# szabodabo/CUDA-MPI-Reductions

Measured on AMD Instinct MI355X. Metric: reduction bandwidth (GB/s, whole node), 1B-double sum at 1/2/4/8 MI355X, higher is better.
Workload: dtype fp64; 1 GPU; global_batch=1000000000, seq_len=1, parallelism=dp1, backend=nccl, n_total_elements=1000000000, op=SUM, collective=fused, launch=graph (chunk 871, 1 replays)

## Files before the change

### csrc/include/mireduce/direct.hpp

```cpp
#pragma once

#include <hip/hip_runtime_api.h>

#include <array>
#include <cstddef>
#include <cstdint>
#include <vector>

#include "mireduce/types.hpp"
#include "mireduce/xrank.hpp"

namespace mireduce {

constexpr int kMaxDirectRanks = 16;
constexpr int kMaxDirectBlocks = 1024;
constexpr int kDirectBlock = 512;
constexpr int kDirectPhases = 3;

struct DirectDesc {
  const char* in[kMaxDirectRanks];
  char* out[kMaxDirectRanks];
  unsigned* sig[kMaxDirectRanks];
  unsigned* ctl;
  int rank;
  int world;
  uint64_t timeout_ticks;
};

class DirectAllreduce {
 public:
  DirectAllreduce(int device, size_t bytes, int grid = 0, double timeout_s = 10.0);
  ~DirectAllreduce();
  DirectAllreduce(const DirectAllreduce&) = delete;
  DirectAllreduce& operator=(const DirectAllreduce&) = delete;

  static constexpr size_t kHandleBytes = 3 * sizeof(IpcHandleBytes) + sizeof(int32_t);
  std::vector<char> handles() const;
  void connect(int rank, int world, const std::vector<std::vector<char>>& all);

  void* in() const { return in_; }
  void* out() const { return out_; }
  size_t bytes() const { return bytes_; }
  int grid() const { return grid_; }
  int rank() const { return rank_; }
  int world() const { return world_; }
  bool connected() const { return connected_; }

  void allreduce(size_t count, DType t, Op op, hipStream_t s);
  void reduce(size_t count, DType t, Op op, int root, hipStream_t s);
  void read_peers(size_t bytes_each, hipStream_t s);
  unsigned error() const;
  unsigned epoch() const;

 private:
  void launch(size_t count, DType t, Op op, int gather_rank, hipStream_t s);
  int device_ = 0, rank_ = 0, world_ = 1, grid_ = 0;
  size_t bytes_ = 0;
  double timeout_s_ = 10.0;
  bool connected_ = false;
  void* in_ = nullptr;
  void* out_ = nullptr;
  unsigned* sig_ = nullptr;
  unsigned* ctl_ = nullptr;
  DirectDesc* desc_ = nullptr;
  uint32_t* sink_ = nullptr;
  std::vector<void*> opened_;
  std::vector<const void*> peer_in_;
};

void direct_chunk(size_t count, size_t elem_size, int world, int r, size_t* begin, size_t* end);

}
```

### csrc/kernels/direct.hip

```cpp
#include <hip/hip_runtime.h>

#include <algorithm>
#include <cstdint>
#include <cstring>

#include "mireduce/check.hpp"
#include "mireduce/direct.hpp"
#include "mireduce/peer.hpp"
#include "mireduce/ops.hpp"

namespace mireduce {
namespace kern {

__device__ __forceinline__ void peer_barrier(const DirectDesc* d, int phase, unsigned e, unsigned err,
                                             bool release) {
  asm volatile("s_waitcnt vmcnt(0)" ::: "memory");
  __syncthreads();
  if (threadIdx.x < 64) {
    const int lane = threadIdx.x;
    if (release) __builtin_amdgcn_fence(__ATOMIC_RELEASE, "");
    const int world = d->world;
    const uint64_t slot = (static_cast<uint64_t>(phase) * kMaxDirectBlocks + blockIdx.x) * kMaxDirectRanks;
    if (lane < world) {
      __hip_atomic_store(d->sig[lane] + slot + d->rank, e, __ATOMIC_RELAXED, __HIP_MEMORY_SCOPE_SYSTEM);
      const unsigned* mine = d->sig[d->rank] + slot + lane;
      const uint64_t limit = err ? 0 : d->timeout_ticks;
      const uint64_t t0 = static_cast<uint64_t>(wall_clock64());
      while (__hip_atomic_load(mine, __ATOMIC_RELAXED, __HIP_MEMORY_SCOPE_SYSTEM) != e) {
        if (static_cast<uint64_t>(wall_clock64()) - t0 > limit) {
          __hip_atomic_fetch_or(d->ctl + 1, 1u, __ATOMIC_RELAXED, __HIP_MEMORY_SCOPE_AGENT);
          break;
        }
        __builtin_amdgcn_s_sleep(1);
      }
    }
    __builtin_amdgcn_fence(__ATOMIC_ACQUIRE, "");
  }
  __syncthreads();
}

__device__ __forceinline__ void block_range(uint64_t nvec, uint64_t* v0, uint64_t* v1) {
  const uint64_t per = (nvec + gridDim.x - 1) / gridDim.x;
  *v0 = std::min<uint64_t>(nvec, blockIdx.x * per);
  *v1 = std::min<uint64_t>(nvec, *v0 + per);
}

template <class T>
__device__ __forceinline__ uint64_t chunk_elems(uint64_t count, int world) {
  constexpr uint64_t N = 16 / sizeof(T);
  const uint64_t per = (count + world - 1) / world;
  return (per + N - 1) / N * N;
}

template <int W>
constexpr int direct_unroll() {
  return W >= 4 ? 1 : (W >= 2 ? 2 : 4);
}

template <class OpT, class T, int W>
__global__ __launch_bounds__(kDirectBlock) void direct_kernel(const DirectDesc* __restrict__ d, uint64_t count,
                                                               int gather_rank) {
  constexpr int N = 16 / sizeof(T);
  constexpr int U = W > 0 ? direct_unroll<W>() : 1;
  using V = T __attribute__((ext_vector_type(N)));
  __shared__ unsigned s_epoch, s_err;
  if (threadIdx.x == 0) {
    s_epoch = __hip_atomic_load(d->ctl, __ATOMIC_RELAXED, __HIP_MEMORY_SCOPE_AGENT) + 1u;
    s_err = __hip_atomic_load(d->ctl + 1, __ATOMIC_RELAXED, __HIP_MEMORY_SCOPE_AGENT);
  }
  __syncthreads();
  const unsigned e = s_epoch;
  const int world = W > 0 ? W : d->world;
  const int rank = d->rank;

  peer_barrier(d, 0, e, s_err, true);

  const uint64_t per = chunk_elems<T>(count, world);
  const uint64_t perv = per / N;
  uint64_t v0, v1;
  block_range(perv, &v0, &v1);
  {
    const uint64_t cb = std::min<uint64_t>(count, rank * per);
    const uint64_t ce = std::min<uint64_t>(count, cb + per);
    const uint64_t nvec = (ce - cb) / N;
    const uint64_t r1 = std::min(v1, nvec);
    T* out = reinterpret_cast<T*>(d->out[rank]);
    if constexpr (W > 0) {
      for (uint64_t i0 = v0 + threadIdx.x; i0 < r1; i0 += U * kDirectBlock) {
        V v[U][W];
#pragma unroll
        for (int u = 0; u < U; ++u) {
          const uint64_t i = i0 + static_cast<uint64_t>(u) * kDirectBlock;
          if (i < r1)
#pragma unroll
            for (int p = 0; p < W; ++p)
              v[u][p] = __builtin_nontemporal_load(reinterpret_cast<const V*>(d->in[p]) + cb / N + i);
        }
#pragma unroll
        for (int u = 0; u < U; ++u) {
          const uint64_t i = i0 + static_cast<uint64_t>(u) * kDirectBlock;
          if (i >= r1) continue;
          V acc = v[u][0];
#pragma unroll
          for (int p = 1; p < W; ++p)
#pragma unroll
            for (int k = 0; k < N; ++k) acc[k] = OpT::apply(acc[k], v[u][p][k]);
          reinterpret_cast<V*>(out)[cb / N + i] = acc;
        }
      }
    } else {
      for (uint64_t i = v0 + threadIdx.x; i < r1; i += kDirectBlock) {
        const uint64_t off = cb / N + i;
        V acc = __builtin_nontemporal_load(reinterpret_cast<const V*>(d->in[0]) + off);
        for (int p = 1; p < world; ++p) {
          const V v = __builtin_nontemporal_load(reinterpret_cast<const V*>(d->in[p]) + off);
#pragma unroll
          for (int k = 0; k < N; ++k) acc[k] = OpT::apply(acc[k], v[k]);
        }
        reinterpret_cast<V*>(out)[off] = acc;
      }
    }
    if (blockIdx.x == gridDim.x - 1) {
      for (uint64_t i = cb + nvec * N + threadIdx.x; i < ce; i += kDirectBlock) {
        T acc = reinterpret_cast<const T*>(d->in[0])[i];
        for (int p = 1; p < world; ++p) acc = OpT::apply(acc, reinterpret_cast<const T*>(d->in[p])[i]);
        out[i] = acc;
      }
    }
  }

  peer_barrier(d, 1, e, s_err, true);

  if (gather_rank < 0 || gather_rank == rank) {
    T* mine = reinterpret_cast<T*>(d->out[rank]);
    if constexpr (W > 0) {
      uint64_t nv[W];
#pragma unroll
      for (int p = 0; p < W; ++p) {
        const uint64_t b = std::min<uint64_t>(count, p * per);
        nv[p] = p == rank ? 0 : (std::min<uint64_t>(count, b + per) - b) / N;
      }
      for (uint64_t i0 = v0 + threadIdx.x; i0 < v1; i0 += U * kDirectBlock) {
        V v[U][W];
#pragma unroll
        for (int u = 0; u < U; ++u) {
          const uint64_t i = i0 + static_cast<uint64_t>(u) * kDirectBlock;
#pragma unroll
          for (int p = 0; p < W; ++p)
            if (i < v1 && i < nv[p])
              v[u][p] = __builtin_nontemporal_load(reinterpret_cast<const V*>(d->out[p]) + p * perv + i);
        }
#pragma unroll
        for (int u = 0; u < U; ++u) {
          const uint64_t i = i0 + static_cast<uint64_t>(u) * kDirectBlock;
#pragma unroll
          for (int p = 0; p < W; ++p)
            if (i < v1 && i < nv[p]) reinterpret_cast<V*>(mine)[p * perv + i] = v[u][p];
        }
      }
    } else {
      for (int p = 0; p < world; ++p) {
        if (p == rank) continue;
        const uint64_t b = std::min<uint64_t>(count, p * per);
        const uint64_t n = (std::min<uint64_t>(count, b + per) - b) / N;
        const uint64_t e1 = std::min(v1, n);
        for (uint64_t i = v0 + threadIdx.x; i < e1; i += kDirectBlock)
          reinterpret_cast<V*>(mine)[p * perv + i] = __builtin_nontemporal_load(reinterpret_cast<const V*>(d->out[p]) + p * perv + i);
      }
    }
    if (blockIdx.x == gridDim.x - 1) {
      for (int p = 0; p < world; ++p) {
        if (p == rank) continue;
        const uint64_t b = std::min<uint64_t>(count, p * per);
        const uint64_t e1 = std::min<uint64_t>(count, b + per);
        for (uint64_t i = b + (e1 - b) / N * N + threadIdx.x; i < e1; i += kDirectBlock)
          mine[i] = reinterpret_cast<const T*>(d->out[p])[i];
      }
    }
  }

  peer_barrier(d, 2, e, s_err, false);
  if (threadIdx.x == 0) {
    const unsigned prev = __hip_atomic_fetch_add(d->ctl + 2, 1u, __ATOMIC_RELAXED, __HIP_MEMORY_SCOPE_AGENT);
    if (prev == gridDim.x - 1) {
      __hip_atomic_store(d->ctl + 2, 0u, __ATOMIC_RELAXED, __HIP_MEMORY_SCOPE_AGENT);
      __hip_atomic_store(d->ctl, e, __ATOMIC_RELAXED, __HIP_MEMORY_SCOPE_AGENT);
    }
  }
}

}

void direct_chunk(size_t count, size_t elem_size, int world, int r, size_t* begin, size_t* end) {
  const size_t vec = 16 / elem_size;
  size_t per = (count + world - 1) / world;
  per = (per + vec - 1) / vec * vec;
  *begin = std::min(count, static_cast<size_t>(r) * per);
  *end = std::min(count, static_cast<size_t>(r + 1) * per);
}

namespace {

struct DeviceGuard {
  int prev = 0;
  explicit DeviceGuard(int dev) {
    MIREDUCE_HIP_THROW(hipGetDevice(&prev));
    MIREDUCE_HIP_THROW(hipSetDevice(dev));
  }
  ~DeviceGuard() { (void)hipSetDevice(prev); }
};

constexpr size_t kSigBytes = static_cast<size_t>(kDirectPhases) * kMaxDirectBlocks * kMaxDirectRanks * sizeof(unsigned);

using DirectFn = void (*)(const DirectDesc*, uint64_t, int, int, hipStream_t);

template <class OpT, class T, int W>
void launch_w(const DirectDesc* d, uint64_t count, int gather, int grid, hipStream_t s) {
  hipLaunchKernelGGL((kern::direct_kernel<OpT, T, W>), dim3(grid), dim3(kDirectBlock), 0, s, d, count, gather);
}

template <class OpT, class T>
DirectFn pick_world(int world) {
  switch (world) {
    case 1: return launch_w<OpT, T, 1>;
    case 2: return launch_w<OpT, T, 2>;
    case 3: return launch_w<OpT, T, 3>;
    case 4: return launch_w<OpT, T, 4>;
    case 5: return launch_w<OpT, T, 5>;
    case 6: return launch_w<OpT, T, 6>;
    case 7: return launch_w<OpT, T, 7>;
    case 8: return launch_w<OpT, T, 8>;
    default: return launch_w<OpT, T, 0>;
  }
}

template <class OpT>
DirectFn pick_type(DType t, int world) {
  switch (t) {
    case DType::Int32: return pick_world<OpT, int32_t>(world);
    case DType::Int64: return pick_world<OpT, int64_t>(world);
    case DType::Float32: return pick_world<OpT, float>(world);
    case DType::Float64: return pick_world<OpT, double>(world);
    default: MIREDUCE_REQUIRE(false, "direct: int32, int64, float32 or float64 only");
  }
  return nullptr;
}

}

DirectAllreduce::DirectAllreduce(int device, size_t bytes, int grid, double timeout_s) : timeout_s_(timeout_s) {
  MIREDUCE_REQUIRE(timeout_s > 0, "direct: timeout must be positive");
  if (device < 0) MIREDUCE_HIP_THROW(hipGetDevice(&device));
  device_ = device;
  DeviceGuard g(device_);
  int cus = 0;
  MIREDUCE_HIP_THROW(hipDeviceGetAttribute(&cus, hipDeviceAttributeMultiprocessorCount, device_));
  grid_ = grid > 0 ? grid : std::max(1, cus);
  MIREDUCE_REQUIRE(grid_ <= kMaxDirectBlocks, "direct: grid exceeds kMaxDirectBlocks");
  bytes_ = (std::max<size_t>(bytes, 16) + 255) / 256 * 256;
  MIREDUCE_HIP_THROW(hipExtMallocWithFlags(&in_, bytes_, hipDeviceMallocFinegrained));
  MIREDUCE_HIP_THROW(hipExtMallocWithFlags(&out_, bytes_, hipDeviceMallocFinegrained));
  MIREDUCE_HIP_THROW(hipExtMallocWithFlags(reinterpret_cast<void**>(&sig_), kSigBytes, hipDeviceMallocUncached));
  MIREDUCE_HIP_THROW(hipMemset(sig_, 0, kSigBytes));
  MIREDUCE_HIP_THROW(hipMalloc(reinterpret_cast<void**>(&ctl_), 256));
  MIREDUCE_HIP_THROW(hipMemset(ctl_, 0, 256));
  MIREDUCE_HIP_THROW(hipMalloc(reinterpret_cast<void**>(&desc_), sizeof(DirectDesc)));
  MIREDUCE_HIP_THROW(hipDeviceSynchronize());
}

DirectAllreduce::~DirectAllreduce() {
  DeviceGuard g(device_);
  for (void* p : opened_) (void)hipIpcCloseMemHandle(p);
  (void)hipFree(sink_);
  (void)hipFree(desc_);
  (void)hipFree(ctl_);
  (void)hipFree(sig_);
  (void)hipFree(out_);
  (void)hipFree(in_);
  (void)hipGetLastError();
}

std::vector<char> DirectAllreduce::handles() const {
  std::vector<char> h(kHandleBytes);
  void* bufs[3] = {in_, out_, sig_};
  for (int k = 0; k < 3; ++k) {
    hipIpcMemHandle_t m;
    MIREDUCE_HIP_THROW(hipIpcGetMemHandle(&m, bufs[k]));
    std::memcpy(h.data() + k * sizeof(IpcHandleBytes), &m, sizeof m);
  }
  const int32_t gr = grid_;
  std::memcpy(h.data() + 3 * sizeof(IpcHandleBytes), &gr, sizeof gr);
  return h;
}

void DirectAllreduce::connect(int rank, int world, const std::vector<std::vector<char>>& all) {
  MIREDUCE_REQUIRE(!connected_, "direct: already connected");
  MIREDUCE_REQUIRE(world >= 1 && world <= kMaxDirectRanks, "direct: world must be 1..16");
  MIREDUCE_REQUIRE(rank >= 0 && rank < world, "direct: rank out of range");
  MIREDUCE_REQUIRE(all.size() == static_cast<size_t>(world), "direct: one handle set per rank");
  DeviceGuard g(device_);
  DirectDesc d{};
  for (int r = 0; r < world; ++r) {
    MIREDUCE_REQUIRE(all[r].size() == kHandleBytes, "direct: bad handle size");
    int32_t gr = 0;
    std::memcpy(&gr, all[r].data() + 3 * sizeof(IpcHandleBytes), sizeof gr);
    MIREDUCE_REQUIRE(gr == grid_, "direct: every rank must use the same grid");
    if (r == rank) {
      d.in[r] = static_cast<const char*>(in_);
      d.out[r] = static_cast<char*>(out_);
      d.sig[r] = sig_;
      continue;
    }
    void* p[3] = {nullptr, nullptr, nullptr};
    for (int k = 0; k < 3; ++k) {
      hipIpcMemHandle_t m;
      std::memcpy(&m, all[r].data() + k * sizeof(IpcHandleBytes), sizeof m);
      MIREDUCE_HIP_THROW(hipIpcOpenMemHandle(&p[k], m, hipIpcMemLazyEnablePeerAccess));
      opened_.push_back(p[k]);
    }
    d.in[r] = static_cast<const char*>(p[0]);
    peer_in_.push_back(p[0]);
    d.out[r] = static_cast<char*>(p[1]);
    d.sig[r] = static_cast<unsigned*>(p[2]);
  }
  d.ctl = ctl_;
  d.rank = rank;
  d.world = world;
  int khz = 0;
  if (hipDeviceGetAttribute(&khz, hipDeviceAttributeWallClockRate, device_) != hipSuccess || khz <= 0) khz = 100000;
  d.timeout_ticks = static_cast<uint64_t>(timeout_s_ * 1e3 * khz);
  MIREDUCE_HIP_THROW(hipMemcpy(desc_, &d, sizeof d, hipMemcpyHostToDevice));
  MIREDUCE_HIP_THROW(hipDeviceSynchronize());
  rank_ = rank;
  world_ = world;
  connected_ = true;
}

void DirectAllreduce::launch(size_t count, DType t, Op op, int gather_rank, hipStream_t s) {
  MIREDUCE_REQUIRE(connected_, "direct: connect() first");
  MIREDUCE_REQUIRE(count * dtype_size(t) <= bytes_, "direct: count exceeds the registered buffers");
  DirectFn fn = nullptr;
  switch (op) {
    case Op::Sum: fn = pick_type<SumOp>(t, world_); break;
    case Op::Min: fn = pick_type<MinOp>(t, world_); break;
    case Op::Max: fn = pick_type<MaxOp>(t, world_); break;
    default: MIREDUCE_REQUIRE(false, "direct: SUM, MIN or MAX");
  }
  (void)hipGetLastError();
  fn(desc_, count, gather_rank, grid_, s);
  MIREDUCE_HIP_THROW(hipGetLastError());
}

void DirectAllreduce::allreduce(size_t count, DType t, Op op, hipStream_t s) { launch(count, t, op, -1, s); }

void DirectAllreduce::reduce(size_t count, DType t, Op op, int root, hipStream_t s) {
  MIREDUCE_REQUIRE(root >= 0 && root < world_, "direct: root out of range");
  launch(count, t, op, root, s);
}

void DirectAllreduce::read_peers(size_t bytes_each, hipStream_t s) {
  MIREDUCE_REQUIRE(connected_, "direct: connect() first");
  MIREDUCE_REQUIRE(bytes_each <= bytes_, "direct: read_peers beyond the registered buffers");
  DeviceGuard g(device_);
  PeerSources src{};
  int n = 0;
  if (peer_in_.empty()) src.p[n++] = in_;
  for (const void* p : peer_in_) src.p[n++] = p;
  const int grid = 128 * n;
  if (!sink_) MIREDUCE_HIP_THROW(hipMalloc(reinterpret_cast<void**>(&sink_), 128 * kMaxPeerSources * sizeof(uint32_t)));
  peer_read(src, n, bytes_each, sink_, grid, s);
}
// ... 17 lines not shown
```

### csrc/python/module.cpp

```cpp
#include <pybind11/pybind11.h>
#include <pybind11/stl.h>

#include <hip/hip_runtime_api.h>

#include <cstdint>
#include <cstring>
#include <memory>

#include "mireduce/arg_reduce.hpp"
#include "mireduce/check.hpp"
#include "mireduce/cpu_reference.hpp"
#include "mireduce/direct.hpp"
#include "mireduce/final_line.hpp"
#include "mireduce/ladder.hpp"
#include "mireduce/moments.hpp"
#include "mireduce/mt19937.hpp"
#include "mireduce/reduce.hpp"
#include "mireduce/reduce_dim.hpp"
#include "mireduce/reduce_many.hpp"
#include "mireduce/scan.hpp"
#include "mireduce/trace.hpp"
#include "mireduce/types.hpp"
#include "mireduce/version.hpp"
#include "mireduce/xrank.hpp"
// ... 78 lines not shown

  m.def("stream_capture_status", [](uintptr_t stream) {
    hipStreamCaptureStatus st = hipStreamCaptureStatusNone;
    const hipError_t e = hipStreamIsCapturing(as_stream(stream), &st);
    if (e != hipSuccess) (void)hipGetLastError();
    return static_cast<int>(st);
  });
  m.def("end_capture", [](uintptr_t stream) {
    hipGraph_t g = nullptr;
    const hipError_t e = hipStreamEndCapture(as_stream(stream), &g);
    if (g) (void)hipGraphDestroy(g);
    (void)hipGetLastError();
    return e == hipSuccess ? std::string() : std::string(hipGetErrorName(e));
  });

  m.def("device_count", [] {
    int n = 0;
    if (hipGetDeviceCount(&n) != hipSuccess) return 0;
    return n;
  });

  m.def("device_info", [](int dev) {
    hipDeviceProp_t p;
    check_hip(hipGetDeviceProperties(&p, dev), "hipGetDeviceProperties");
    py::dict d;
    d["name"] = std::string(p.name);
    d["arch"] = std::string(p.gcnArchName);
    d["cus"] = p.multiProcessorCount;
    d["total_mem"] = static_cast<uint64_t>(p.totalGlobalMem);
    d["clock_khz"] = p.clockRate;
    d["mem_clock_khz"] = p.memoryClockRate;
    d["mem_bus_width"] = p.memoryBusWidth;
    d["l2_bytes"] = p.l2CacheSize;
    d["pci_bus_id"] = p.pciBusID;
    int rt = 0;
    (void)hipRuntimeGetVersion(&rt);
    d["hip_runtime"] = rt;
    return d;
  });

  m.def("mem_info", [](int dev) {
    int prev = 0;
    check_hip(hipGetDevice(&prev), "hipGetDevice");
    check_hip(hipSetDevice(dev), "hipSetDevice");
    size_t free_b = 0, total_b = 0;
    check_hip(hipMemGetInfo(&free_b, &total_b), "hipMemGetInfo");
    check_hip(hipSetDevice(prev), "hipSetDevice");
    return py::make_tuple(free_b, total_b);
  });

  py::class_<Workspace, std::shared_ptr<Workspace>>(m, "Workspace")
      .def(py::init<int, int>(), py::arg("device") = -1, py::arg("max_grid") = 16384)
      .def_property_readonly("device", &Workspace::device)
      .def_property_readonly("num_cus", &Workspace::num_cus)
      .def_property_readonly("max_grid", &Workspace::max_grid)
      .def_property_readonly("partials_ptr", [](const Workspace& w) { return reinterpret_cast<uintptr_t>(w.partials()); })
      .def("reset", [](Workspace& w, uintptr_t stream) { w.reset(as_stream(stream)); }, py::arg("stream") = 0)
      .def("error", &Workspace::error)
      .def_property_readonly("fan_ptr", [](const Workspace& w) { return reinterpret_cast<uintptr_t>(w.fan()); });

  py::class_<BoundReduce>(m, "BoundReduce")
      .def(py::init([](Workspace& ws, uintptr_t in, uint64_t n, int dtype, int op, int acc, uintptr_t out,
                       int block, int unroll, int wg_per_cu, int max_blocks, int policy,
                       bool single_pass, uintptr_t xrank, int window, int xcd_skew,
                       int64_t segment_bytes) {
             ReduceConfig cfg = make_cfg(block, unroll, wg_per_cu, max_blocks, policy, single_pass,
                                         window, xcd_skew, segment_bytes);
             cfg.xrank = as_ptr<const void>(xrank);
             return new BoundReduce(as_ptr<const void>(in), n, static_cast<DType>(dtype), static_cast<Op>(op),
                                    static_cast<DType>(acc), as_ptr<void>(out), ws, cfg);
           }),
           py::arg("ws"), py::arg("in_ptr"), py::arg("n"), py::arg("dtype"), py::arg("op"), py::arg("acc"),
           py::arg("out_ptr"), py::arg("block") = 0, py::arg("unroll") = 0, py::arg("wg_per_cu") = 0,
           py::arg("max_blocks") = 0, py::arg("policy") = -1,
           py::arg("single_pass") = true, py::arg("xrank") = 0, py::arg("window") = -1,
           py::arg("xcd_skew") = kSkewAuto, py::arg("segment_bytes") = 0,
           py::keep_alive<1, 2>())
      .def("launch", [](const BoundReduce& b, uintptr_t stream, uintptr_t out) { b.launch(as_stream(stream), as_ptr<void>(out)); },
           py::arg("stream"), py::arg("out_ptr") = 0)
      .def_property_readonly("plan", [](const BoundReduce& b) { return plan_dict(b.plan()); })
      .def("error", &BoundReduce::error);

  py::class_<XrankChannel, std::shared_ptr<XrankChannel>>(m, "XrankChannel")
      .def(py::init<int, double>(), py::arg("device") = -1, py::arg("timeout_s") = 2.0)
      .def("handle", [](const XrankChannel& c) {
        const IpcHandleBytes h = c.handle();
        return py::bytes(h.data(), h.size());
      })
      .def("connect", [](XrankChannel& c, int rank, int world, const std::vector<py::bytes>& handles) {
        std::vector<IpcHandleBytes> hs(handles.size());
        for (size_t i = 0; i < handles.size(); ++i) {
          const std::string s = handles[i];
          if (s.size() != sizeof(IpcHandleBytes)) throw Error("XrankChannel.connect: bad handle size");
          std::memcpy(hs[i].data(), s.data(), s.size());
        }
        c.connect(rank, world, hs);
      }, py::arg("rank"), py::arg("world"), py::arg("handles"))
      .def_property_readonly("connected", &XrankChannel::connected)
      .def_property_readonly("desc_ptr", [](const XrankChannel& c) { return reinterpret_cast<uintptr_t>(c.device_desc()); })
      .def_property_readonly("rank", &XrankChannel::rank)
      .def_property_readonly("world", &XrankChannel::world)
      .def("error", &XrankChannel::error)
      .def("epoch", &XrankChannel::epoch)
      .def("clear_error", &XrankChannel::clear_error)
      .def("set_stamps", [](XrankChannel& c, uintptr_t p, unsigned cap) { c.set_stamps(as_ptr<uint64_t>(p), cap); },
           py::arg("stamps_ptr"), py::arg("cap"))
      .def_property_readonly("ticks_per_us", &XrankChannel::ticks_per_us);
  m.attr("XRANK_MAX_RANKS") = kMaxXrankRanks;

  m.def("arm_final_line", [](const std::string& line) { arm_final_line(line); }, py::arg("line"));
  m.def("disarm_final_line", &disarm_final_line);
  m.def("emit_final_line", [](const std::string& line) {
    py::gil_scoped_release nogil;
    return emit_final_line(line);
  }, py::arg("line"));
  m.def("final_line_emitted", &final_line_emitted);

  m.def("memcpy_d2d", [](uintptr_t dst, uintptr_t src, uint64_t bytes, uintptr_t stream) {
    check_hip(hipMemcpyAsync(as_ptr<void>(dst), as_ptr<const void>(src), bytes, hipMemcpyDeviceToDevice,
                             as_stream(stream)), "hipMemcpyAsync");
  }, py::arg("dst"), py::arg("src"), py::arg("bytes"), py::arg("stream") = 0);

  py::class_<DirectAllreduce, std::shared_ptr<DirectAllreduce>>(m, "DirectAllreduce")
      .def(py::init<int, size_t, int, double>(), py::arg("device") = -1, py::arg("bytes") = 16,
           py::arg("grid") = 0, py::arg("timeout_s") = 10.0)
      .def("handles", [](const DirectAllreduce& d) {
        const std::vector<char> h = d.handles();
        return py::bytes(h.data(), h.size());
      })
      .def("connect", [](DirectAllreduce& d, int rank, int world, const std::vector<py::bytes>& all) {
        std::vector<std::vector<char>> hs;
        for (const auto& b : all) {
          const std::string s = b;
          hs.emplace_back(s.begin(), s.end());
        }
        d.connect(rank, world, hs);
      }, py::arg("rank"), py::arg("world"), py::arg("handles"))
      .def_property_readonly("in_ptr", [](const DirectAllreduce& d) { return reinterpret_cast<uintptr_t>(d.in()); })
      .def_property_readonly("out_ptr", [](const DirectAllreduce& d) { return reinterpret_cast<uintptr_t>(d.out()); })
      .def_property_readonly("bytes", &DirectAllreduce::bytes)
      .def_property_readonly("grid", &DirectAllreduce::grid)
      .def_property_readonly("connected", &DirectAllreduce::connected)
      .def("allreduce", [](DirectAllreduce& d, uint64_t count, int dtype, int op, uintptr_t stream) {
        d.allreduce(count, static_cast<DType>(dtype), static_cast<Op>(op), as_stream(stream));
      }, py::arg("count"), py::arg("dtype"), py::arg("op"), py::arg("stream") = 0)
      .def("reduce", [](DirectAllreduce& d, uint64_t count, int dtype, int op, int root, uintptr_t stream) {
        d.reduce(count, static_cast<DType>(dtype), static_cast<Op>(op), root, as_stream(stream));
      }, py::arg("count"), py::arg("dtype"), py::arg("op"), py::arg("root") = 0, py::arg("stream") = 0)
      .def("read_peers", [](DirectAllreduce& d, uint64_t bytes_each, uintptr_t stream) {
        d.read_peers(bytes_each, as_stream(stream));
      })
      .def("error", &DirectAllreduce::error)
      .def("epoch", &DirectAllreduce::epoch);

  m.def(
      "reduce",
      [](Workspace& ws, uintptr_t in, uint64_t n, int dtype, int op, int acc, uintptr_t out,
         uintptr_t stream, int block, int unroll, int wg_per_cu, int max_blocks,
         int policy, bool single_pass, uint64_t fanin_bound_ticks, int debug_delay_wg,
         uint64_t debug_delay_ticks, int window, uintptr_t xrank, uintptr_t wg_stamps, int xcd_skew,
         uint64_t debug_delay_anchor_ticks, int64_t segment_bytes) {
        ReduceConfig cfg = make_cfg(block, unroll, wg_per_cu, max_blocks, policy, single_pass, window,
                                    xcd_skew, segment_bytes);
        cfg.xrank = as_ptr<const void>(xrank);
        cfg.debug_wg_stamps = as_ptr<uint64_t>(wg_stamps);
        cfg.fanin_bound_ticks = fanin_bound_ticks;
        cfg.debug_delay_wg = debug_delay_wg;
        cfg.debug_delay_ticks = debug_delay_ticks;
        cfg.debug_delay_anchor_ticks = debug_delay_anchor_ticks;
        const LaunchPlan p = reduce(as_ptr<const void>(in), n, static_cast<DType>(dtype),
                                    static_cast<Op>(op), static_cast<DType>(acc),
                                    as_ptr<void>(out), ws, as_stream(stream), cfg);
        return plan_dict(p);
      },
      py::arg("ws"), py::arg("in_ptr"), py::arg("n"), py::arg("dtype"), py::arg("op"),
      py::arg("acc"), py::arg("out_ptr"), py::arg("stream") = 0, py::arg("block") = 0,
      py::arg("unroll") = 0, py::arg("wg_per_cu") = 0, py::arg("max_blocks") = 0,
      py::arg("policy") = -1, py::arg("single_pass") = true,
      py::arg("fanin_bound_ticks") = 0, py::arg("debug_delay_wg") = -1,
      py::arg("debug_delay_ticks") = 0, py::arg("window") = -1, py::arg("xrank") = 0, py::arg("wg_stamps") = 0,
      py::arg("xcd_skew") = kSkewAuto, py::arg("debug_delay_anchor_ticks") = 0, py::arg("segment_bytes") = 0);

  m.def(
      "plan",
      [](uintptr_t in, uint64_t n, int dtype, int num_cus, int max_grid, int block, int unroll,
         int wg_per_cu, int max_blocks, int policy, bool single_pass, int window,
         int op, int xcd_skew, int64_t segment_bytes) {
        MIREDUCE_REQUIRE(op >= 0 && op < kNumOps, "op out of range");
        const ReduceConfig cfg = make_cfg(block, unroll, wg_per_cu, max_blocks, policy, single_pass,
                                          window, xcd_skew, segment_bytes);
        LaunchPlan p = plan_reduce(as_ptr<const void>(in), n, static_cast<DType>(dtype), cfg, num_cus, max_grid,
                                   static_cast<Op>(op));
        plan_segmentation(n, static_cast<DType>(dtype), cfg, p, std::min(256, max_grid));
        return plan_dict(p);
      },
      py::arg("in_ptr"), py::arg("n"), py::arg("dtype"), py::arg("num_cus") = 256,
      py::arg("max_grid") = 16384, py::arg("block") = 0, py::arg("unroll") = 0,
      py::arg("wg_per_cu") = 0, py::arg("max_blocks") = 0,
      py::arg("policy") = -1, py::arg("single_pass") = true, py::arg("window") = -1,
      py::arg("op") = 0, py::arg("xcd_skew") = kSkewAuto, py::arg("segment_bytes") = 0);

  m.def(
      "reduce_partials",
      [](uintptr_t in, uint64_t n, int dtype, int op, int acc, uintptr_t partials, int max_grid,
         int num_cus, uintptr_t stream, int block, int unroll, int wg_per_cu, int max_blocks, int policy) {
        ReduceConfig c = make_cfg(block, unroll, wg_per_cu, max_blocks, policy, false);
        return plan_dict(reduce_partials(as_ptr<const void>(in), n, static_cast<DType>(dtype),
                                         static_cast<Op>(op), static_cast<DType>(acc),
                                         as_ptr<void>(partials), max_grid, num_cus,
                                         as_stream(stream), c));
      },
      py::arg("in_ptr"), py::arg("n"), py::arg("dtype"), py::arg("op"), py::arg("acc"),
      py::arg("partials_ptr"), py::arg("max_grid"), py::arg("num_cus"), py::arg("stream") = 0,
      py::arg("block") = 0, py::arg("unroll") = 0, py::arg("wg_per_cu") = 0,
      py::arg("max_blocks") = 0, py::arg("policy") = -1);

  m.def(
      "reduce_finalize",
      [](uintptr_t partials, uint64_t count, int acc, int op, uintptr_t out, uintptr_t stream) {
        reduce_finalize(as_ptr<const void>(partials), count, static_cast<DType>(acc),
                        static_cast<Op>(op), as_ptr<void>(out), as_stream(stream));
      },
      py::arg("partials_ptr"), py::arg("count"), py::arg("acc"), py::arg("op"), py::arg("out_ptr"),
      py::arg("stream") = 0);

  m.def(
      "combine_elementwise",
      [](uintptr_t inout, uintptr_t other, uint64_t n, int dtype, int op, uintptr_t stream) {
        combine_elementwise(as_ptr<void>(inout), as_ptr<const void>(other), n,
                            static_cast<DType>(dtype), static_cast<Op>(op), as_stream(stream));
      },
      py::arg("inout_ptr"), py::arg("other_ptr"), py::arg("n"), py::arg("dtype"), py::arg("op"),
      py::arg("stream") = 0);

  m.def(
      "fill_device",
      [](uintptr_t ptr, uint64_t n, int dtype, int pattern, uint64_t seed, uint64_t offset,
         double value, uintptr_t stream) {
        FillSpec s;
        s.pattern = static_cast<Pattern>(pattern);
        s.seed = seed;
        s.offset = offset;
        s.value = value;
        fill_device(as_ptr<void>(ptr), n, static_cast<DType>(dtype), s, as_stream(stream));
      },
      py::arg("ptr"), py::arg("n"), py::arg("dtype"), py::arg("pattern") = 0,
      py::arg("seed") = 0x5EED, py::arg("offset") = 0, py::arg("value") = 0.0,
      py::arg("stream") = 0);

  m.def(
      "fill_host",
      [](uintptr_t ptr, uint64_t n, int dtype, int pattern, uint64_t seed, uint64_t offset,
         double value) {
        FillSpec s;
        s.pattern = static_cast<Pattern>(pattern);
        s.seed = seed;
        s.offset = offset;
        s.value = value;
        py::gil_scoped_release nogil;
        fill_host(as_ptr<void>(ptr), n, static_cast<DType>(dtype), s);
      },
      py::arg("ptr"), py::arg("n"), py::arg("dtype"), py::arg("pattern") = 0,
      py::arg("seed") = 0x5EED, py::arg("offset") = 0, py::arg("value") = 0.0);

  m.def(
      "cpu_reduce",
      [](uintptr_t ptr, uint64_t n, int dtype, int op, int acc, int threads) {
        alignas(8) unsigned char out[8] = {0};
        {
          py::gil_scoped_release nogil;
          cpu_reduce(as_ptr<const void>(ptr), n, static_cast<DType>(dtype), static_cast<Op>(op),
                     static_cast<DType>(acc), out, threads);
        }
        return acc_to_py(out, static_cast<DType>(acc));
      },
      py::arg("ptr"), py::arg("n"), py::arg("dtype"), py::arg("op"), py::arg("acc"),
      py::arg("threads") = 0);

  m.def(
      "cpu_abs_sum",
      [](uintptr_t ptr, uint64_t n, int dtype, int threads) {
        py::gil_scoped_release nogil;
        return cpu_abs_sum(as_ptr<const void>(ptr), n, static_cast<DType>(dtype), threads);
      },
      py::arg("ptr"), py::arg("n"), py::arg("dtype"), py::arg("threads") = 0);

  m.def("sum_tolerance", [](int dtype, int acc, uint64_t n, double abs_sum) {
    return sum_tolerance(static_cast<DType>(dtype), static_cast<DType>(acc), n, abs_sum);
  });

  m.def("default_acc", [](int dtype, int op) {
    return static_cast<int>(default_acc(static_cast<DType>(dtype), static_cast<Op>(op)));
  });

  m.def("acc_supported", [](int dtype, int op, int acc) {
    return acc_supported(static_cast<DType>(dtype), static_cast<Op>(op), static_cast<DType>(acc));
  });

  m.def(
      "ladder_reduce",
      [](int kernel, uintptr_t in, uint64_t n, int dtype, int op, int acc, uintptr_t out, uintptr_t scratch,
         int threads, int max_blocks, uintptr_t stream) {
        return ladder_reduce(kernel, as_ptr<const void>(in), n, static_cast<DType>(dtype), static_cast<Op>(op),
                             static_cast<DType>(acc), as_ptr<void>(out), as_ptr<void>(scratch), threads, max_blocks,
                             as_stream(stream));
      },
// ... 244 lines not shown
```

Before: 7368 GB/s.

## Restructure direct allreduce into tiled, software-pipelined streaming with per-world plans

Rewrites the direct allreduce kernel's reduce and gather phases into a tile-based streaming loop. Each wave owns contiguous tiles addressed with 32-bit voffset plus immediate offsets, and a rolling window of loads is kept in flight ahead of the stores, with sched_barriers fixing the instruction order. A per-world plan picks block size, unroll and window; world 1 now uses 256-thread blocks with a deeper unroll. Tiles are assigned round-robin across blocks instead of contiguous block ranges, and partial tiles are handled by an edge path. This aims for more memory-level parallelism and less address arithmetic, at the cost of higher register pressure and more complex tail handling.

```diff
diff --git a/csrc/include/mireduce/direct.hpp b/csrc/include/mireduce/direct.hpp
--- a/csrc/include/mireduce/direct.hpp
+++ b/csrc/include/mireduce/direct.hpp
@@ -70,4 +70,7 @@
 
 void direct_chunk(size_t count, size_t elem_size, int world, int r, size_t* begin, size_t* end);
 
+bool direct_plan_of(int world, int* block, int* unroll, int* window);
+size_t direct_tile_elems(int world, size_t elem_size);
+
 }
diff --git a/csrc/kernels/direct.hip b/csrc/kernels/direct.hip
--- a/csrc/kernels/direct.hip
+++ b/csrc/kernels/direct.hip
@@ -4,192 +4,12 @@
 #include <cstdint>
 #include <cstring>
 
+#include "direct_kernels.hpp"
 #include "mireduce/check.hpp"
 #include "mireduce/direct.hpp"
 #include "mireduce/peer.hpp"
-#include "mireduce/ops.hpp"
 
 namespace mireduce {
-namespace kern {
-
-__device__ __forceinline__ void peer_barrier(const DirectDesc* d, int phase, unsigned e, unsigned err,
-                                             bool release) {
-  asm volatile("s_waitcnt vmcnt(0)" ::: "memory");
-  __syncthreads();
-  if (threadIdx.x < 64) {
-    const int lane = threadIdx.x;
-    if (release) __builtin_amdgcn_fence(__ATOMIC_RELEASE, "");
-    const int world = d->world;
-    const uint64_t slot = (static_cast<uint64_t>(phase) * kMaxDirectBlocks + blockIdx.x) * kMaxDirectRanks;
-    if (lane < world) {
-      __hip_atomic_store(d->sig[lane] + slot + d->rank, e, __ATOMIC_RELAXED, __HIP_MEMORY_SCOPE_SYSTEM);
-      const unsigned* mine = d->sig[d->rank] + slot + lane;
-      const uint64_t limit = err ? 0 : d->timeout_ticks;
-      const uint64_t t0 = static_cast<uint64_t>(wall_clock64());
-      while (__hip_atomic_load(mine, __ATOMIC_RELAXED, __HIP_MEMORY_SCOPE_SYSTEM) != e) {
-        if (static_cast<uint64_t>(wall_clock64()) - t0 > limit) {
-          __hip_atomic_fetch_or(d->ctl + 1, 1u, __ATOMIC_RELAXED, __HIP_MEMORY_SCOPE_AGENT);
-          break;
-        }
-        __builtin_amdgcn_s_sleep(1);
-      }
-    }
-    __builtin_amdgcn_fence(__ATOMIC_ACQUIRE, "");
-  }
-  __syncthreads();
-}
-
-__device__ __forceinline__ void block_range(uint64_t nvec, uint64_t* v0, uint64_t* v1) {
-  const uint64_t per = (nvec + gridDim.x - 1) / gridDim.x;
-  *v0 = std::min<uint64_t>(nvec, blockIdx.x * per);
-  *v1 = std::min<uint64_t>(nvec, *v0 + per);
-}
-
-template <class T>
-__device__ __forceinline__ uint64_t chunk_elems(uint64_t count, int world) {
-  constexpr uint64_t N = 16 / sizeof(T);
-  const uint64_t per = (count + world - 1) / world;
-  return (per + N - 1) / N * N;
-}
-
-template <int W>
-constexpr int direct_unroll() {
-  return W >= 4 ? 1 : (W >= 2 ? 2 : 4);
-}
-
-template <class OpT, class T, int W>
-__global__ __launch_bounds__(kDirectBlock) void direct_kernel(const DirectDesc* __restrict__ d, uint64_t count,
-                                                               int gather_rank) {
-  constexpr int N = 16 / sizeof(T);
-  constexpr int U = W > 0 ? direct_unroll<W>() : 1;
-  using V = T __attribute__((ext_vector_type(N)));
-  __shared__ unsigned s_epoch, s_err;
-  if (threadIdx.x == 0) {
-    s_epoch = __hip_atomic_load(d->ctl, __ATOMIC_RELAXED, __HIP_MEMORY_SCOPE_AGENT) + 1u;
-    s_err = __hip_atomic_load(d->ctl + 1, __ATOMIC_RELAXED, __HIP_MEMORY_SCOPE_AGENT);
-  }
-  __syncthreads();
-  const unsigned e = s_epoch;
-  const int world = W > 0 ? W : d->world;
-  const int rank = d->rank;
-
-  peer_barrier(d, 0, e, s_err, true);
-
-  const uint64_t per = chunk_elems<T>(count, world);
-  const uint64_t perv = per / N;
-  uint64_t v0, v1;
-  block_range(perv, &v0, &v1);
-  {
-    const uint64_t cb = std::min<uint64_t>(count, rank * per);
-    const uint64_t ce = std::min<uint64_t>(count, cb + per);
-    const uint64_t nvec = (ce - cb) / N;
-    const uint64_t r1 = std::min(v1, nvec);
-    T* out = reinterpret_cast<T*>(d->out[rank]);
-    if constexpr (W > 0) {
-      for (uint64_t i0 = v0 + threadIdx.x; i0 < r1; i0 += U * kDirectBlock) {
-        V v[U][W];
-#pragma unroll
-        for (int u = 0; u < U; ++u) {
-          const uint64_t i = i0 + static_cast<uint64_t>(u) * kDirectBlock;
-          if (i < r1)
-#pragma unroll
-            for (int p = 0; p < W; ++p)
-              v[u][p] = __builtin_nontemporal_load(reinterpret_cast<const V*>(d->in[p]) + cb / N + i);
-        }
-#pragma unroll
-        for (int u = 0; u < U; ++u) {
-          const uint64_t i = i0 + static_cast<uint64_t>(u) * kDirectBlock;
-          if (i >= r1) continue;
-          V acc = v[u][0];
-#pragma unroll
-          for (int p = 1; p < W; ++p)
-#pragma unroll
-            for (int k = 0; k < N; ++k) acc[k] = OpT::apply(acc[k], v[u][p][k]);
-          reinterpret_cast<V*>(out)[cb / N + i] = acc;
-        }
-      }
-    } else {
-      for (uint64_t i = v0 + threadIdx.x; i < r1; i += kDirectBlock) {
-        const uint64_t off = cb / N + i;
-        V acc = __builtin_nontemporal_load(reinterpret_cast<const V*>(d->in[0]) + off);
-        for (int p = 1; p < world; ++p) {
-          const V v = __builtin_nontemporal_load(reinterpret_cast<const V*>(d->in[p]) + off);
-#pragma unroll
-          for (int k = 0; k < N; ++k) acc[k] = OpT::apply(acc[k], v[k]);
-        }
-        reinterpret_cast<V*>(out)[off] = acc;
-      }
-    }
-    if (blockIdx.x == gridDim.x - 1) {
-      for (uint64_t i = cb + nvec * N + threadIdx.x; i < ce; i += kDirectBlock) {
-        T acc = reinterpret_cast<const T*>(d->in[0])[i];
-        for (int p = 1; p < world; ++p) acc = OpT::apply(acc, reinterpret_cast<const T*>(d->in[p])[i]);
-        out[i] = acc;
-      }
-    }
-  }
-
-  peer_barrier(d, 1, e, s_err, true);
-
-  if (gather_rank < 0 || gather_rank == rank) {
-    T* mine = reinterpret_cast<T*>(d->out[rank]);
-    if constexpr (W > 0) {
-      uint64_t nv[W];
-#pragma unroll
-      for (int p = 0; p < W; ++p) {
-        const uint64_t b = std::min<uint64_t>(count, p * per);
-        nv[p] = p == rank ? 0 : (std::min<uint64_t>(count, b + per) - b) / N;
-      }
-      for (uint64_t i0 = v0 + threadIdx.x; i0 < v1; i0 += U * kDirectBlock) {
-        V v[U][W];
-#pragma unroll
-        for (int u = 0; u < U; ++u) {
-          const uint64_t i = i0 + static_cast<uint64_t>(u) * kDirectBlock;
-#pragma unroll
-          for (int p = 0; p < W; ++p)
-            if (i < v1 && i < nv[p])
-              v[u][p] = __builtin_nontemporal_load(reinterpret_cast<const V*>(d->out[p]) + p * perv + i);
-        }
-#pragma unroll
-        for (int u = 0; u < U; ++u) {
-          const uint64_t i = i0 + static_cast<uint64_t>(u) * kDirectBlock;
-#pragma unroll
-          for (int p = 0; p < W; ++p)
-            if (i < v1 && i < nv[p]) reinterpret_cast<V*>(mine)[p * perv + i] = v[u][p];
-        }
-      }
-    } else {
-      for (int p = 0; p < world; ++p) {
-        if (p == rank) continue;
-        const uint64_t b = std::min<uint64_t>(count, p * per);
-        const uint64_t n = (std::min<uint64_t>(count, b + per) - b) / N;
-        const uint64_t e1 = std::min(v1, n);
-        for (uint64_t i = v0 + threadIdx.x; i < e1; i += kDirectBlock)
-          reinterpret_cast<V*>(mine)[p * perv + i] = __builtin_nontemporal_load(reinterpret_cast<const V*>(d->out[p]) + p * perv + i);
-      }
-    }
-    if (blockIdx.x == gridDim.x - 1) {
-      for (int p = 0; p < world; ++p) {
-        if (p == rank) continue;
-        const uint64_t b = std::min<uint64_t>(count, p * per);
-        const uint64_t e1 = std::min<uint64_t>(count, b + per);
-        for (uint64_t i = b + (e1 - b) / N * N + threadIdx.x; i < e1; i += kDirectBlock)
-          mine[i] = reinterpret_cast<const T*>(d->out[p])[i];
-      }
-    }
-  }
-
-  peer_barrier(d, 2, e, s_err, false);
-  if (threadIdx.x == 0) {
-    const unsigned prev = __hip_atomic_fetch_add(d->ctl + 2, 1u, __ATOMIC_RELAXED, __HIP_MEMORY_SCOPE_AGENT);
-    if (prev == gridDim.x - 1) {
-      __hip_atomic_store(d->ctl + 2, 0u, __ATOMIC_RELAXED, __HIP_MEMORY_SCOPE_AGENT);
-      __hip_atomic_store(d->ctl, e, __ATOMIC_RELAXED, __HIP_MEMORY_SCOPE_AGENT);
-    }
-  }
-}
-
-}
 
 void direct_chunk(size_t count, size_t elem_size, int world, int r, size_t* begin, size_t* end) {
   const size_t vec = 16 / elem_size;
@@ -199,6 +19,29 @@
   *end = std::min(count, static_cast<size_t>(r + 1) * per);
 }
 
+bool direct_plan_of(int world, int* block, int* unroll, int* window) {
+  kern::DirectPlan p{};
+  switch (world) {
+    case 1: p = kern::direct_plan<1>(); break;
+    case 2: p = kern::direct_plan<2>(); break;
+    case 3: p = kern::direct_plan<3>(); break;
+    case 4: p = kern::direct_plan<4>(); break;
+    case 5: p = kern::direct_plan<5>(); break;
+    case 6: p = kern::direct_plan<6>(); break;
+    case 7: p = kern::direct_plan<7>(); break;
+    case 8: p = kern::direct_plan<8>(); break;
+    default: return false;
+  }
+  *block = p.block, *unroll = p.unroll, *window = p.window;
+  return true;
+}
+
+size_t direct_tile_elems(int world, size_t elem_size) {
+  int block = 0, unroll = 0, window = 0;
+  if (!direct_plan_of(world, &block, &unroll, &window)) return 0;
+  return static_cast<size_t>(block) * unroll * (16 / elem_size);
+}
+
 namespace {
 
 struct DeviceGuard {
@@ -216,7 +59,8 @@
 
 template <class OpT, class T, int W>
 void launch_w(const DirectDesc* d, uint64_t count, int gather, int grid, hipStream_t s) {
-  hipLaunchKernelGGL((kern::direct_kernel<OpT, T, W>), dim3(grid), dim3(kDirectBlock), 0, s, d, count, gather);
+  hipLaunchKernelGGL((kern::direct_kernel<OpT, T, W>), dim3(grid), dim3(kern::direct_plan<W>().block), 0, s, d, count,
+                     gather);
 }
 
 template <class OpT, class T>
diff --git a/csrc/kernels/direct_kernels.hpp b/csrc/kernels/direct_kernels.hpp
--- /dev/null
+++ b/csrc/kernels/direct_kernels.hpp
@@ -0,0 +1,298 @@
+#pragma once
+
+#include <hip/hip_runtime.h>
+
+#include <algorithm>
+#include <cstdint>
+#include <type_traits>
+
+#include "mireduce/direct.hpp"
+#include "mireduce/ops.hpp"
+
+namespace mireduce {
+namespace kern {
+
+__device__ __forceinline__ void peer_barrier(const DirectDesc* d, int phase, unsigned e, unsigned err,
+                                             bool release) {
+  asm volatile("s_waitcnt vmcnt(0)" ::: "memory");
+  __syncthreads();
+  if (threadIdx.x < 64) {
+    const int lane = threadIdx.x;
+    if (release) __builtin_amdgcn_fence(__ATOMIC_RELEASE, "");
+    const int world = d->world;
+    const uint64_t slot = (static_cast<uint64_t>(phase) * kMaxDirectBlocks + blockIdx.x) * kMaxDirectRanks;
+    if (lane < world) {
+      __hip_atomic_store(d->sig[lane] + slot + d->rank, e, __ATOMIC_RELAXED, __HIP_MEMORY_SCOPE_SYSTEM);
+      const unsigned* mine = d->sig[d->rank] + slot + lane;
+      const uint64_t limit = err ? 0 : d->timeout_ticks;
+      const uint64_t t0 = static_cast<uint64_t>(wall_clock64());
+      while (__hip_atomic_load(mine, __ATOMIC_RELAXED, __HIP_MEMORY_SCOPE_SYSTEM) != e) {
+        if (static_cast<uint64_t>(wall_clock64()) - t0 > limit) {
+          __hip_atomic_fetch_or(d->ctl + 1, 1u, __ATOMIC_RELAXED, __HIP_MEMORY_SCOPE_AGENT);
+          break;
+        }
+        __builtin_amdgcn_s_sleep(1);
+      }
+    }
+    __builtin_amdgcn_fence(__ATOMIC_ACQUIRE, "");
+  }
+  __syncthreads();
+}
+
+__device__ __forceinline__ void block_range(uint64_t nvec, uint64_t* v0, uint64_t* v1) {
+  const uint64_t per = (nvec + gridDim.x - 1) / gridDim.x;
+  *v0 = std::min<uint64_t>(nvec, blockIdx.x * per);
+  *v1 = std::min<uint64_t>(nvec, *v0 + per);
+}
+
+template <class T>
+__device__ __forceinline__ uint64_t chunk_elems(uint64_t count, int world) {
+  constexpr uint64_t N = 16 / sizeof(T);
+  const uint64_t per = (count + world - 1) / world;
+  return (per + N - 1) / N * N;
+}
+
+template <class V>
+using GlobalPtr = V __attribute__((address_space(1)))*;
+
+constexpr int kWaveVecBytes = 64 * 16;
+
+template <class V>
+__device__ __forceinline__ V direct_load(GlobalPtr<const char> base, uint32_t voff, int imm) {
+  return __builtin_nontemporal_load(reinterpret_cast<GlobalPtr<const V>>(base + voff + imm));
+}
+
+template <bool NT, class V>
+__device__ __forceinline__ void direct_store(GlobalPtr<char> base, uint32_t voff, int imm, const V& v) {
+  const GlobalPtr<V> p = reinterpret_cast<GlobalPtr<V>>(base + voff + imm);
+  if constexpr (NT) __builtin_nontemporal_store(v, p);
+  else *p = v;
+}
+
+template <class OpT, class T, int S, bool COPY, int BLOCK, int U, int WIN, bool NTST>
+__device__ __forceinline__ void stream_tiles(const char* const (&src)[S], char* const (&dst)[COPY ? S : 1],
+                                             uint32_t t0, uint32_t step, uint32_t n) {
+  static_assert(WIN >= 1 && U % WIN == 0, "the window must divide the unroll");
+  static_assert(BLOCK % 64 == 0 && U * kWaveVecBytes <= 8192, "a position's offset must fit the immediate");
+  constexpr int N = 16 / sizeof(T);
+  constexpr int D = COPY ? S : 1;
+  using V = T __attribute__((ext_vector_type(N)));
+  constexpr uint64_t kTileBytes = static_cast<uint64_t>(BLOCK) * U * 16;
+  constexpr int kBias = U * kWaveVecBytes > 4096 ? 4096 : 0;
+  if (n == 0) return;
+  const uint32_t voff = (threadIdx.x / 64) * (U * kWaveVecBytes) + (threadIdx.x % 64) * 16;
+  const uint64_t adv = step * kTileBytes;
+  GlobalPtr<const char> ps[S];
+  GlobalPtr<char> pd[D];
+#pragma unroll
+  for (int p = 0; p < S; ++p) ps[p] = (GlobalPtr<const char>)src[p] + (t0 * kTileBytes + kBias);
+#pragma unroll
+  for (int p = 0; p < D; ++p) pd[p] = (GlobalPtr<char>)dst[p] + (t0 * kTileBytes + kBias);
+  V buf[WIN][S];
+#pragma unroll
+  for (int j = 0; j < WIN; ++j) {
+#pragma unroll
+    for (int p = 0; p < S; ++p) buf[j][p] = direct_load<V>(ps[p], voff, j * kWaveVecBytes - kBias);
+    __builtin_amdgcn_sched_barrier(0);
+  }
+  auto tile = [&](auto more) {
+    constexpr bool kMore = decltype(more)::value;
+#pragma unroll
+    for (int u = 0; u < U; ++u) {
+      const int at = u * kWaveVecBytes - kBias;
+      if constexpr (COPY) {
+#pragma unroll
+        for (int p = 0; p < S; ++p) direct_store<NTST>(pd[p], voff, at, buf[u % WIN][p]);
+      } else {
+        V acc = buf[u % WIN][0];
+#pragma unroll
+        for (int p = 1; p < S; ++p)
+#pragma unroll
+          for (int k = 0; k < N; ++k) acc[k] = OpT::apply(acc[k], buf[u % WIN][p][k]);
+        direct_store<NTST>(pd[0], voff, at, acc);
+      }
+      const int j = u + WIN;
+      if (j < U) {
+#pragma unroll
+        for (int p = 0; p < S; ++p) buf[u % WIN][p] = direct_load<V>(ps[p], voff, j * kWaveVecBytes - kBias);
+      } else if constexpr (kMore) {
+#pragma unroll
+        for (int p = 0; p < S; ++p)
+          buf[u % WIN][p] = direct_load<V>(ps[p] + adv, voff, (j - U) * kWaveVecBytes - kBias);
+      }
+      __builtin_amdgcn_sched_barrier(0);
+    }
+    if constexpr (kMore) {
+#pragma unroll
+      for (int p = 0; p < S; ++p) ps[p] += adv;
+#pragma unroll
+      for (int p = 0; p < D; ++p) pd[p] += adv;
+    }
+  };
+#pragma nounroll
+  for (; n > 1; --n) tile(std::true_type{});
+  tile(std::false_type{});
+}
+
+template <class OpT, class T, int S, bool COPY, int BLOCK>
+__device__ __forceinline__ void edge_vectors(const char* const (&src)[S], char* const (&dst)[COPY ? S : 1],
+                                             uint64_t i0, uint64_t i1, const uint64_t (&lim)[S]) {
+  constexpr int N = 16 / sizeof(T);
+  using V = T __attribute__((ext_vector_type(N)));
+  for (uint64_t i = i0 + threadIdx.x; i < i1; i += BLOCK) {
+    if constexpr (COPY) {
+#pragma unroll
+      for (int p = 0; p < S; ++p)
+        if (i < lim[p]) ((GlobalPtr<V>)dst[p])[i] = __builtin_nontemporal_load((GlobalPtr<const V>)src[p] + i);
+    } else {
+      if (i >= lim[0]) continue;
+      V acc = __builtin_nontemporal_load((GlobalPtr<const V>)src[0] + i);
+#pragma unroll
+      for (int p = 1; p < S; ++p) {
+        const V v = __builtin_nontemporal_load((GlobalPtr<const V>)src[p] + i);
+#pragma unroll
+        for (int k = 0; k < N; ++k) acc[k] = OpT::apply(acc[k], v[k]);
+      }
+      ((GlobalPtr<V>)dst[0])[i] = acc;
+    }
+  }
+}
+
+template <class OpT, class T, int S, bool COPY, int BLOCK, int U, int WIN, bool NTST>
+__device__ __forceinline__ void stream_phase(const char* const (&src)[S], char* const (&dst)[COPY ? S : 1],
+                                             const uint64_t (&lim)[S], uint64_t perv) {
+  constexpr uint64_t kTile = static_cast<uint64_t>(BLOCK) * U;
+  uint64_t lo = lim[0], hi = lim[0];
+#pragma unroll
+  for (int p = 1; p < S; ++p) lo = std::min(lo, lim[p]), hi = std::max(hi, lim[p]);
+  const uint32_t nfull = static_cast<uint32_t>(lo / kTile), b = blockIdx.x, grid = gridDim.x;
+  const uint32_t n = b < nfull ? (nfull - 1 - b) / grid + 1 : 0;
+  stream_tiles<OpT, T, S, COPY, BLOCK, U, WIN, NTST>(src, dst, b, grid, n);
+  hi = std::min(hi, perv);
+  for (uint64_t t = b + static_cast<uint64_t>(n) * grid; t * kTile < hi; t += grid)
+    edge_vectors<OpT, T, S, COPY, BLOCK>(src, dst, t * kTile, std::min(hi, (t + 1) * kTile), lim);
+}
+
+struct DirectPlan {
+  int block, unroll, window;
+  bool nt_store;
+};
+
+template <int W>
+constexpr DirectPlan direct_plan() {
+  return W >= 4 ? DirectPlan{kDirectBlock, 4, 2, false}
+                : (W >= 2 ? DirectPlan{kDirectBlock, 4, 4, false} : DirectPlan{256, 8, 8, false});
+}
+
+template <class OpT, class T, int W, int BLOCK, int U, int WIN, bool NTST>
+__device__ __forceinline__ void direct_body(const DirectDesc* __restrict__ d, uint64_t count, int gather_rank) {
+  constexpr int N = 16 / sizeof(T);
+  using V = T __attribute__((ext_vector_type(N)));
+  __shared__ unsigned s_epoch, s_err;
+  if (threadIdx.x == 0) {
+    s_epoch = __hip_atomic_load(d->ctl, __ATOMIC_RELAXED, __HIP_MEMORY_SCOPE_AGENT) + 1u;
+    s_err = __hip_atomic_load(d->ctl + 1, __ATOMIC_RELAXED, __HIP_MEMORY_SCOPE_AGENT);
+  }
+  __syncthreads();
+  const unsigned e = s_epoch;
+  const int world = W > 0 ? W : d->world;
+  const int rank = d->rank;
+
+  peer_barrier(d, 0, e, s_err, true);
+
+  const uint64_t per = chunk_elems<T>(count, world);
+  const uint64_t perv = per / N;
+  uint64_t v0 = 0, v1 = 0;
+  if constexpr (W == 0) block_range(perv, &v0, &v1);
+  {
+    const uint64_t cb = std::min<uint64_t>(count, rank * per);
+    const uint64_t ce = std::min<uint64_t>(count, cb + per);
+    const uint64_t nvec = (ce - cb) / N;
+    T* out = reinterpret_cast<T*>(d->out[rank]);
+    if constexpr (W > 0) {
+      const char* src[W];
+      uint64_t lim[W];
+#pragma unroll
+      for (int p = 0; p < W; ++p) src[p] = d->in[p] + cb * sizeof(T), lim[p] = nvec;
+      char* const dst[1] = {d->out[rank] + cb * sizeof(T)};
+      stream_phase<OpT, T, W, false, BLOCK, U, WIN, NTST>(src, dst, lim, perv);
+    } else {
+      const uint64_t r1 = std::min(v1, nvec);
+      for (uint64_t i = v0 + threadIdx.x; i < r1; i += BLOCK) {
+        const uint64_t off = cb / N + i;
+        V acc = __builtin_nontemporal_load(reinterpret_cast<const V*>(d->in[0]) + off);
+        for (int p = 1; p < world; ++p) {
+          const V v = __builtin_nontemporal_load(reinterpret_cast<const V*>(d->in[p]) + off);
+#pragma unroll
+          for (int k = 0; k < N; ++k) acc[k] = OpT::apply(acc[k], v[k]);
+        }
+        reinterpret_cast<V*>(out)[off] = acc;
+      }
+    }
+    if (blockIdx.x == gridDim.x - 1) {
+      for (uint64_t i = cb + nvec * N + threadIdx.x; i < ce; i += BLOCK) {
+        T acc = reinterpret_cast<const T*>(d->in[0])[i];
+        for (int p = 1; p < world; ++p) acc = OpT::apply(acc, reinterpret_cast<const T*>(d->in[p])[i]);
+        out[i] = acc;
+      }
+    }
+  }
+
+  peer_barrier(d, 1, e, s_err, true);
+
+  if (gather_rank < 0 || gather_rank == rank) {
+    T* mine = reinterpret_cast<T*>(d->out[rank]);
+    if constexpr (W > 1) {
+      const char* src[W - 1];
+      char* dst[W - 1];
+      uint64_t lim[W - 1];
+#pragma unroll
+      for (int k = 0; k < W - 1; ++k) {
+        const int p = k + (k >= rank);
+        const uint64_t b = std::min<uint64_t>(count, p * per);
+        lim[k] = (std::min<uint64_t>(count, b + per) - b) / N;
+        src[k] = d->out[p] + p * per * sizeof(T);
+        dst[k] = d->out[rank] + p * per * sizeof(T);
+      }
+      stream_phase<OpT, T, W - 1, true, BLOCK, U, WIN, NTST>(src, dst, lim, perv);
+    } else if constexpr (W == 0) {
+      for (int p = 0; p < world; ++p) {
+        if (p == rank) continue;
+        const uint64_t b = std::min<uint64_t>(count, p * per);
+        const uint64_t n = (std::min<uint64_t>(count, b + per) - b) / N;
+        const uint64_t e1 = std::min(v1, n);
+        for (uint64_t i = v0 + threadIdx.x; i < e1; i += BLOCK)
+          reinterpret_cast<V*>(mine)[p * perv + i] = __builtin_nontemporal_load(reinterpret_cast<const V*>(d->out[p]) + p * perv + i);
+      }
+    }
+    if (blockIdx.x == gridDim.x - 1) {
+      for (int p = 0; p < world; ++p) {
+        if (p == rank) continue;
+        const uint64_t b = std::min<uint64_t>(count, p * per);
+        const uint64_t e1 = std::min<uint64_t>(count, b + per);
+        for (uint64_t i = b + (e1 - b) / N * N + threadIdx.x; i < e1; i += BLOCK)
+          mine[i] = reinterpret_cast<const T*>(d->out[p])[i];
+      }
+    }
+  }
+
+  peer_barrier(d, 2, e, s_err, false);
+  if (threadIdx.x == 0) {
+    const unsigned prev = __hip_atomic_fetch_add(d->ctl + 2, 1u, __ATOMIC_RELAXED, __HIP_MEMORY_SCOPE_AGENT);
+    if (prev == gridDim.x - 1) {
+      __hip_atomic_store(d->ctl + 2, 0u, __ATOMIC_RELAXED, __HIP_MEMORY_SCOPE_AGENT);
+      __hip_atomic_store(d->ctl, e, __ATOMIC_RELAXED, __HIP_MEMORY_SCOPE_AGENT);
+    }
+  }
+}
+
+template <class OpT, class T, int W>
+__global__ __launch_bounds__(kDirectBlock) void direct_kernel(const DirectDesc* __restrict__ d, uint64_t count,
+                                                               int gather_rank) {
+  constexpr DirectPlan kPlan = direct_plan<W>();
+  static_assert(kPlan.block <= kDirectBlock);
+  direct_body<OpT, T, W, kPlan.block, kPlan.unroll, kPlan.window, kPlan.nt_store>(d, count, gather_rank);
+}
+
+}
+}
diff --git a/csrc/python/module.cpp b/csrc/python/module.cpp
--- a/csrc/python/module.cpp
+++ b/csrc/python/module.cpp
@@ -254,6 +254,12 @@
       })
       .def("error", &DirectAllreduce::error)
       .def("epoch", &DirectAllreduce::epoch);
+  m.def("direct_tile_elems", &direct_tile_elems, py::arg("world"), py::arg("elem_size"));
+  m.def("direct_plan", [](int world) {
+    int block = 0, unroll = 0, window = 0;
+    if (!direct_plan_of(world, &block, &unroll, &window)) throw std::invalid_argument("direct_plan: world must be 1..8");
+    return py::make_tuple(block, unroll, window);
+  }, py::arg("world"));
 
   m.def(
       "reduce",
```

Result: no change. 7337 GB/s (-0.4%).
